# ghnmqdtg/VM-ASR

Hardware: AMD Instinct MI355X
Metric: audio clips/sec (train step) 48kHz n_fft=1024 (higher is better)
Workload: dtype bf16 (autocast over G; scan/STFT f32; MPD f32/bf16x3 MFMA); 1 GPU; vm_asr_48k_MPD.yaml full train step, DIMS 16 d_state 1 n_fft 1024 clip 122640@48k; per_gpu_batch=4, global_batch=4, parallelism=dp1, execution=hipGraph replay, 2 streams, generator_streams=2

## Files before the change

### include/vmasr_hip.h

```cpp
#ifndef VMASR_HIP_H
#define VMASR_HIP_H

#include <stddef.h>
#include <stdint.h>

#ifdef __cplusplus
extern "C" {
#endif

#define VMASR_ABI_VERSION 1

typedef void *vmasr_stream_t;

enum { VMASR_F32 = 0, VMASR_F16 = 1, VMASR_BF16 = 2 };

enum {
    VMASR_OK = 0,
    VMASR_EINVAL = -1,
    VMASR_EALIGN = -2,
    VMASR_ENOSPACE = -3
};

int vmasr_abi_version(void);
const char *vmasr_last_error(void);
// ... 149 lines not shown
                           int32_t k, int32_t stride, int32_t pad, int64_t rows, int32_t dtype, vmasr_stream_t stream);
int vmasr_col2im_kx1_stacked(const void *dcols, void *dx, const int64_t *Ns, const int32_t *Hs, int32_t n, int32_t C, int32_t k, int32_t stride,
                             int32_t pad, int64_t rows, int64_t dx_rows, int32_t dtype, vmasr_stream_t stream);
int vmasr_stack_rows(const void *const *srcs, const int64_t *Ms, int32_t n, void *full, int64_t rows, int64_t row_bytes,
                     vmasr_stream_t stream);


int vmasr_bias_gelu_fwd(float *acc, const float *bias, float *act, int32_t slots, int64_t M, int32_t N, int32_t parts,
                        vmasr_stream_t stream);
int vmasr_weight_prep_split(const float *w, void *out, int32_t n, int32_t N, int32_t K, vmasr_stream_t stream);
int vmasr_weight_transpose(const float *w, void *hi, void *lo, float *out32, int32_t n, int32_t N, int32_t Cin, int32_t k,
                           vmasr_stream_t stream);
int vmasr_sum_parts(const float *parts, float *out, int32_t P, int32_t n, int32_t S, int64_t NK, vmasr_stream_t stream);
int vmasr_gelu_bwd_split(const float *pre, const float *g, void *hi, void *lo, void *cat3, float *db, int32_t slots, int64_t M,
                         int32_t N, vmasr_stream_t stream);
int vmasr_gelu_bwd(const float *pre, const float *g, float *gx, float *db, int32_t slots, int64_t M, int32_t N, vmasr_stream_t stream);

typedef struct vmasr_cg_slot {
    const void *ah, *al;
    const void *bh, *bl;
    float *c0;
    float *c1;
    void *ch, *cl;
    const float *bias;
    int64_t nseq;
    int32_t H;
    int32_t reserved;
} vmasr_cg_slot;
int vmasr_conv_mfma_supported(int32_t Cin, int32_t Cout, int32_t k, int32_t stride);
int vmasr_conv_mfma_supported_launch(int32_t Cin, int32_t Cout, int32_t k, int32_t stride, int32_t n, int64_t rows);
int vmasr_conv_mfma_config(int32_t pass, int32_t Cin, int32_t Cout, int32_t ops, int32_t out[3]);
void vmasr_conv_set_cu_limit(int32_t cus);
int32_t vmasr_conv_get_cu_limit(void);
int vmasr_conv_mfma_fwd(const vmasr_cg_slot *slots, int32_t n, int32_t Cin, int32_t Cout, int32_t k, int32_t stride, int32_t pad,
                        int64_t rows_out, int32_t act, vmasr_stream_t stream);
int vmasr_conv_mfma_dgrad(const vmasr_cg_slot *slots, int32_t n, int32_t Cin, int32_t Cout, int32_t k, int32_t stride, int32_t pad,
                          int64_t rows_in, vmasr_stream_t stream);
int vmasr_conv_f32_fwd(const vmasr_cg_slot *slots, int32_t n, int32_t Cin, int32_t Cout, int32_t k, int32_t stride, int32_t pad,
                       int64_t rows_out, int32_t act, vmasr_stream_t stream);
int vmasr_conv_f32_dgrad(const vmasr_cg_slot *slots, int32_t n, int32_t Cin, int32_t Cout, int32_t k, int32_t stride, int32_t pad,
                         int64_t rows_in, vmasr_stream_t stream);
int vmasr_conv_mfma_wgrad(const vmasr_cg_slot *slots, int32_t n, int32_t Cin, int32_t Cout, int32_t k, int32_t stride, int32_t pad,
                          int32_t splits, vmasr_stream_t stream);
typedef struct vmasr_cg_gelu_bwd {
    const float *pre;
    const signed char *sgn;
    int64_t valid;
    float scale;
    int32_t reserved;
    float *db;
} vmasr_cg_gelu_bwd;
int vmasr_conv_mfma_dgrad_gelu(const vmasr_cg_slot *slots, const vmasr_cg_gelu_bwd *epi, const float *gtok, int32_t n, int32_t Cin, int32_t Cout,
                               int32_t k, int32_t stride, int32_t pad, int64_t rows_in, vmasr_stream_t stream);

int vmasr_wgrad_finish_multi(const float *const *parts, float *const *dws, float *const *dbs, float *const *e1s, float *const *e2s,
                             const int32_t *Ss, const int32_t *Ns, const int32_t *Ks, const int32_t *lds, int32_t n, vmasr_stream_t stream);

int vmasr_linear_f64acc(const float *x, const float *w, const float *bias, float *y, int64_t rows, int32_t out_features,
                        int32_t in_features, vmasr_stream_t stream);

typedef struct vmasr_adamw_item {
    float *p;
    const float *g;
    float *m;
    float *v;
    void *lp;
// ... 246 lines not shown
```

### vm_asr_amd/_lib.py

```python
import ctypes
import os

from . import knobs

_HERE = os.path.dirname(os.path.abspath(__file__))
LIB_PATH = knobs.get("VMASR_LIB") or os.path.join(_HERE, "libvmasr_hip.so")

c_i32, c_i64, c_vp, c_sz = ctypes.c_int32, ctypes.c_int64, ctypes.c_void_p, ctypes.c_size_t

F32, F16, BF16 = 0, 1, 2


class SScanParams(ctypes.Structure):
    _fields_ = (
        [(n, c_i32) for n in ("batch", "dim", "seqlen", "dstate", "n_groups", "n_chunks", "dtype",
                              "delta_softplus")]
        + [(n, c_i64) for n in ("A_d_stride", "A_dstate_stride",
                                "B_batch_stride", "B_group_stride", "B_dstate_stride",
                                "C_batch_stride", "C_group_stride", "C_dstate_stride",
                                "u_batch_stride", "u_d_stride", "delta_batch_stride", "delta_d_stride",
                                "out_batch_stride", "out_d_stride")]
        + [(n, c_vp) for n in ("A_ptr", "B_ptr", "C_ptr", "D_ptr", "u_ptr", "delta_ptr",
                               "delta_bias_ptr", "out_ptr", "x_ptr")]
    )
# ... 86 lines not shown
    "vmasr_bias_gelu_fwd": (ctypes.c_int, [c_vp, c_vp, c_vp, c_i32, c_i64, c_i32, c_i32, c_vp]),
    "vmasr_gelu_bwd": (ctypes.c_int, [c_vp, c_vp, c_vp, c_vp, c_i32, c_i64, c_i32, c_vp]),
    "vmasr_sn_dot_blocks": (c_i32, []),
    "vmasr_sn_stack_fwd": (ctypes.c_int, [c_vp, c_vp, c_i32, c_vp, c_vp, c_vp, c_i32, c_i32, c_i32, c_vp]),
    "vmasr_sn_stack_bwd": (ctypes.c_int, [c_vp, c_vp, c_vp, c_vp, c_vp, c_vp, c_i32, c_vp, c_i32, c_i32, c_i32, c_vp]),
    "vmasr_conv_post_supported": (ctypes.c_int, [c_i32, c_i32]),
    "vmasr_conv_post_fwd": (ctypes.c_int, [c_vp, c_vp, c_vp, c_vp, c_vp, c_vp, c_i32, c_i64, c_i32, c_i32, c_vp]),
    "vmasr_conv_post_bwd": (ctypes.c_int, [c_vp, c_vp, c_vp, c_vp, c_vp, c_vp, c_vp, c_vp, c_i32, c_i64, c_i32, c_i32, c_vp]),
    "vmasr_conv_post_bwd_gelu": (ctypes.c_int, [c_vp] * 16 + [c_i32, c_i64, c_i32, c_i32, c_vp]),
    "vmasr_conv_first_fwd": (ctypes.c_int, [c_vp, c_vp, c_vp, c_i32, c_vp, c_vp, c_vp, c_vp, c_i64, c_vp]),
    "vmasr_conv_first_bwd": (ctypes.c_int, [c_vp, c_vp, c_vp, c_i32, c_vp, c_vp, c_vp, c_vp, c_vp, c_vp, c_i64, c_vp]),
    "vmasr_adamw_chunk": (c_i32, []),
    "vmasr_adamw_step": (ctypes.c_int, [c_vp, c_vp, c_i32, c_i64, c_vp, c_vp, ctypes.c_float, ctypes.c_float, ctypes.c_float, c_vp]),
    "vmasr_masked_l1_blocks": (c_i32, []),
    "vmasr_masked_l1_fwd": (ctypes.c_int, [c_vp, c_vp, c_vp, c_vp, c_vp, c_vp, c_i32, c_i64, c_i64, c_i32, c_vp]),
    "vmasr_masked_l1_bwd": (ctypes.c_int, [c_vp, c_vp, c_vp, c_vp, c_vp, c_i32, c_i64, c_i32, c_vp]),
    "vmasr_lsgan_fwd": (ctypes.c_int, [c_vp, c_vp, c_vp, c_i32, c_vp, c_vp]),
    "vmasr_lsgan_bwd": (ctypes.c_int, [c_vp, c_vp, c_vp, c_vp, c_i32, c_vp, c_vp]),
    "vmasr_masked_l1_bwd_add": (ctypes.c_int, [c_vp, c_vp, c_vp, c_vp, c_vp, c_vp, c_i32, c_i64, c_i32, c_vp]),
    "vmasr_sum_parts": (ctypes.c_int, [c_vp, c_vp, c_i32, c_i32, c_i32, c_i64, c_vp]),
    "vmasr_weight_prep_split": (ctypes.c_int, [c_vp, c_vp, c_i32, c_i32, c_i32, c_vp]),
    "vmasr_weight_transpose": (ctypes.c_int, [c_vp, c_vp, c_vp, c_vp, c_i32, c_i32, c_i32, c_i32, c_vp]),
    "vmasr_gelu_bwd_split": (ctypes.c_int, [c_vp, c_vp, c_vp, c_vp, c_vp, c_vp, c_i32, c_i64, c_i32, c_vp]),
    "vmasr_conv_mfma_supported": (ctypes.c_int, [c_i32, c_i32, c_i32, c_i32]),
    "vmasr_conv_mfma_supported_launch": (ctypes.c_int, [c_i32, c_i32, c_i32, c_i32, c_i32, ctypes.c_int64]),
    "vmasr_conv_mfma_config": (ctypes.c_int, [c_i32, c_i32, c_i32, c_i32, ctypes.POINTER(c_i32)]),
    "vmasr_mark_time": (ctypes.c_int, [c_vp, c_vp]),
    "vmasr_im2col2d_rows": (ctypes.c_int, [c_vp, c_vp] + [c_i32] * 10 + [c_vp, c_i32, c_i32, c_vp]),
    "vmasr_col2im2d_rows": (ctypes.c_int, [c_vp, c_vp] + [c_i32] * 10 + [c_vp, c_i32, c_i32, c_vp]),
    "vmasr_skinny_linear_supported": (ctypes.c_int, [c_i64, c_i32, c_i32]),
    "vmasr_skinny_linear": (ctypes.c_int, [c_vp, c_vp, c_vp, c_vp, c_i64, c_i32, c_i32, c_i64, c_i64, c_i32, c_i32, c_vp]),
    "vmasr_conv_set_cu_limit": (None, [c_i32]),
    "vmasr_conv_get_cu_limit": (c_i32, []),
    "vmasr_conv_mfma_fwd": (ctypes.c_int, [ctypes.POINTER(CgSlot), c_i32, c_i32, c_i32, c_i32, c_i32, c_i32, c_i64, c_i32, c_vp]),
    "vmasr_conv_mfma_dgrad": (ctypes.c_int, [ctypes.POINTER(CgSlot), c_i32, c_i32, c_i32, c_i32, c_i32, c_i32, c_i64, c_vp]),
    "vmasr_conv_f32_fwd": (ctypes.c_int, [ctypes.POINTER(CgSlot), c_i32, c_i32, c_i32, c_i32, c_i32, c_i32, c_i64, c_i32, c_vp]),
    "vmasr_conv_f32_dgrad": (ctypes.c_int, [ctypes.POINTER(CgSlot), c_i32, c_i32, c_i32, c_i32, c_i32, c_i32, c_i64, c_vp]),
    "vmasr_conv_mfma_wgrad": (ctypes.c_int, [ctypes.POINTER(CgSlot), c_i32, c_i32, c_i32, c_i32, c_i32, c_i32, c_i32, c_vp]),
    "vmasr_conv_mfma_dgrad_gelu": (ctypes.c_int, [ctypes.POINTER(CgSlot), ctypes.POINTER(CgGeluBwd), c_vp, c_i32, c_i32, c_i32, c_i32, c_i32,
                                                  c_i32, c_i64, c_vp]),
    "vmasr_wgrad_finish_multi": (ctypes.c_int, [c_vp, c_vp, c_vp, c_vp, c_vp, c_vp, c_vp, c_vp, c_vp, c_i32, c_vp]),
    "vmasr_linear_f64acc": (ctypes.c_int, [c_vp, c_vp, c_vp, c_vp, c_i64, c_i32, c_i32, c_vp]),
    "vmasr_ss2d_glue_supported": (ctypes.c_int, [c_i32, c_i32, c_i32]),
    "vmasr_ss2d_pre_fwd": (ctypes.c_int, [c_vp, c_vp, c_vp, c_i32, c_i32, c_i32, c_i32, c_vp]),
    "vmasr_ss2d_pre_bwd": (ctypes.c_int, [c_vp, c_vp, c_vp, c_vp, c_i32, c_i32, c_i32, c_i32, c_vp]),
    "vmasr_ln_gate_fwd": (ctypes.c_int, [c_vp] * 7 + [c_i32, c_i32, c_i32, ctypes.c_float, c_i32, c_vp]),
    "vmasr_ln_gate_bwd": (ctypes.c_int, [c_vp] * 11 + [c_i32, c_i32, c_i32, c_i32, c_vp]),
    "vmasr_ln_gate_bwd_workspace": (c_i64, [c_i32, c_i32, c_i32, c_i32]),
    "vmasr_ln_gate_bwd_ws": (ctypes.c_int, [c_vp] * 12 + [c_i32, c_i32, c_i32, c_i32, c_vp]),
    "vmasr_ln_gate_pair_supported": (ctypes.c_int, [c_i32, c_i32, c_i32]),
    "vmasr_ln_gate_pair_fwd": (ctypes.c_int, [c_vp] * 8 + [c_i32, c_i32, c_i32, c_i32, ctypes.c_float, c_i32, c_vp]),
    "vmasr_ln_gate_pair_bwd": (ctypes.c_int, [c_vp] * 13 + [c_i32, c_i32, c_i32, c_i32, c_i32, c_vp]),
    "vmasr_ss2d_supported": (ctypes.c_int, [c_i32] * 5),
    "vmasr_ss2d_part_floats": (c_sz, [c_i32] * 4),
    "vmasr_ss2d_fwd": (ctypes.c_int, [ctypes.POINTER(SS2DParams), c_vp]),
    "vmasr_ss2d_bwd": (ctypes.c_int, [ctypes.POINTER(SS2DParams), c_vp]),
    "vmasr_ss2d_deep_supported": (ctypes.c_int, [c_i32] * 5),
    "vmasr_ss2d_deep_waves_per_row": (c_i32, [c_i32, c_i32]),
    "vmasr_ss2d_deep_fwd": (ctypes.c_int, [ctypes.POINTER(SS2DDeepParams), c_vp]),
    "vmasr_ss2d_deep_bwd": (ctypes.c_int, [ctypes.POINTER(SS2DDeepParams), c_vp]),
    "vmasr_set_deterministic": (None, [ctypes.c_int]),
    "vmasr_get_deterministic": (ctypes.c_int, []),
    "vmasr_det_timeouts": (ctypes.c_int64, []),
    "vmasr_prof_enable": (None, [ctypes.c_int]),
    "vmasr_prof_reset": (None, []),
    "vmasr_prof_name": (ctypes.c_char_p, [ctypes.c_int]),
# ... 23 lines not shown
    "vmasr_stem1d_time_tile": (c_i32, []),
    "vmasr_stem1d_channel_group": (c_i32, []),
    "vmasr_stem1d_supported": (ctypes.c_int, [c_i32] * 4),
    "vmasr_stem1d_supported_launch": (ctypes.c_int, [c_i32] * 5 + [c_i64]),
    "vmasr_stem1d_bwd_workspace": (c_sz, [c_i32] * 5 + [c_i64]),
    "vmasr_stem1d_fwd": (ctypes.c_int, [c_vp] * 4 + [c_i32] * 2 + [c_i64] + [c_i32] * 4 + [c_vp]),
    "vmasr_stem1d_bwd": (ctypes.c_int, [c_vp] * 8 + [c_sz] + [c_i32] * 2 + [c_i64] + [c_i32] * 4 + [c_vp]),
    "vmasr_resample_poly": (ctypes.c_int, [c_vp, c_vp, c_vp, c_i32, c_i64, c_i64, c_i32, c_i32, c_i32, c_vp]),
    "vmasr_resample_design_workspace": (c_sz, [c_i32]),
    "vmasr_resample_design": (ctypes.c_int, [c_vp, c_i32, c_i32, c_i32, c_vp, c_sz, c_vp]),
    "vmasr_degrade_batch_workspace": (c_sz, [c_vp, c_i32]),
    "vmasr_degrade_batch": (ctypes.c_int, [c_vp, c_vp, c_vp, c_vp, c_i32, c_i64, c_vp, c_sz, c_vp]),
}

_lib = None


def lib():
    global _lib
    if _lib is None:
        if not os.path.exists(LIB_PATH):
            raise RuntimeError(
                f"{LIB_PATH} is missing: build it with `make -C vm_asr_amd/csrc` "
                "(or __graft_entry__.build()). vm_asr_amd has no CPU fallback.")
        import torch
        l = ctypes.CDLL(LIB_PATH)
        for name, (res, args) in SYMBOLS.items():
            fn = getattr(l, name)
            fn.restype, fn.argtypes = res, args
        if l.vmasr_abi_version() != 1:
            raise RuntimeError("libvmasr_hip.so ABI version mismatch")
        if knobs.get("VMASR_DETERMINISTIC"):
            l.vmasr_set_deterministic(1)
        knobs.warn_undeclared()
        _lib = l
    return _lib


def check(code, what):
    if code != 0:
        msg = lib().vmasr_last_error().decode() or "unknown error"
        raise RuntimeError(f"{what} failed ({code}): {msg}")


def torch_dtype_code(dt):
    import torch
    try:
        return {torch.float32: F32, torch.float16: F16, torch.bfloat16: BF16}[dt]
    except KeyError:
        raise RuntimeError(f"unsupported dtype {dt}: expected float32 / float16 / bfloat16")


def det_mode():
    if knobs.get("VMASR_DETERMINISTIC"):
        return True
    try:
        return bool(lib().vmasr_get_deterministic())
    except (OSError, RuntimeError, AttributeError):
        return False


def current_stream(device):
    import torch
    return ctypes.c_void_p(torch.cuda.current_stream(device).cuda_stream)


# ... 94 lines not shown
```

### vm_asr_amd/csrc/convgemm.hip

```cpp
#include <algorithm>
#include <cstdlib>
#include <type_traits>

#include "common.h"

namespace vmasr {
namespace {

typedef __bf16 bf16x8 __attribute__((ext_vector_type(8)));
typedef float f32x16 __attribute__((ext_vector_type(16)));
typedef float f32x4 __attribute__((ext_vector_type(4)));
typedef unsigned u32x4 __attribute__((ext_vector_type(4)));
typedef __attribute__((address_space(1))) const void *cg_gptr;
typedef __attribute__((address_space(3))) void *cg_lptr;
__device__ uint4 cg_zero_page[4];

constexpr int CG_BM = 128, CG_BN = 128, CG_BK = 32;
constexpr int CG_TILE = CG_BM * CG_BK * 2;
constexpr int CG_STAGE = 4 * CG_TILE;
constexpr int CG_MAXP = 24;

struct CgProb {
    const bf16_t *ah, *al, *bh, *bl;
    float *c0, *c1;
// ... 498 lines not shown
                const bf16x8 ah = cw_frag<RBG, 16>(s, 0, wm * WTM + i * 16, lane);
                const bf16x8 al = cw_frag<RBG, 16>(s + TILE_G, 0, wm * WTM + i * 16, lane);
#pragma unroll
                for (int j = 0; j < TJ; ++j) {
                    acc[i][j] = __builtin_amdgcn_mfma_f32_16x16x32_bf16(al, bh[j], acc[i][j], 0, 0, 0);
                    acc[i][j] = __builtin_amdgcn_mfma_f32_16x16x32_bf16(ah, bl[j], acc[i][j], 0, 0, 0);
                    acc[i][j] = __builtin_amdgcn_mfma_f32_16x16x32_bf16(ah, bh[j], acc[i][j], 0, 0, 0);
                }
            }
        }
        if (!MID_STORE && more) CW_STORE(buf ^ 1);
        __syncthreads();
    }
#undef CW_LOAD
#undef CW_STORE

    const int KC = P.k * Cin;
    float *dw = pr.dw + (size_t)split * Cout * KC;
#pragma unroll
    for (int i = 0; i < TI; ++i)
#pragma unroll
        for (int j = 0; j < TJ; ++j) {
            const int col = kc0 + wn * WTN + j * MF + (MF == 32 ? lr : (lane & 15));
#pragma unroll
            for (int r = 0; r < NR; ++r) {
                const int row = co0 + wm * WTM + i * MF + (MF == 32 ? (r & 3) + 8 * (r >> 2) + 4 * lh : 4 * (lane >> 4) + r);
                dw[(size_t)row * KC + col] = acc[i][j][r];
            }
        }
    __syncthreads();
    }
}

}
}

using namespace vmasr;

namespace {

int g_cg_cu_limit = 0;

int cg_grid(int tiles, size_t smem) {
    if (g_cg_cu_limit <= 0) return tiles;
    const int per_cu = std::max(1, (int)((160 * 1024) / std::max<size_t>(smem, 1)));
    static const int slack = [] { const char *e = getenv("VMASR_CONV_CU_SLACK"); return e ? atoi(e) : 24; }();
    const int cap = std::min(256, g_cg_cu_limit + slack) * per_cu;
    const int rounds = (tiles + cap - 1) / cap;
    const int g = ((tiles + rounds - 1) / rounds + 7) / 8 * 8;
    return std::min(tiles, std::min(g, cap));
}

template <int BM, int BN, int WM, int WN, int MF, int OPS = 0>
int cg_launch_cfg(CgParams &P, int epi, hipStream_t st, int kid, double bytes) {
    int tiles = 0;
    P.ntiles_n = P.NB / BN;
    for (int i = 0; i < P.nprob; ++i) {
        P.prob[i].tile_start = tiles;
        P.prob[i].mtiles = (std::max(P.prob[i].M, P.prob[i].zero_rows) + BM - 1) / BM;
        tiles += P.prob[i].mtiles * P.ntiles_n;
    }
    P.total_tiles = tiles;
    if (tiles == 0) return 0;
    constexpr size_t smem = 2 * (2 * BM * 64 + 2 * BN * 64) + BM * sizeof(int);
    constexpr bool HAS_EPI2 = BN >= 128 && OPS == 0;
    static bool attr_done = false;
// ... 23 lines not shown
    static const int v = [] { const char *e = getenv("VMASR_CONV_TILE"); return e ? atoi(e) : 0; }();
    return v;
}
int env_conv_mfma() {
    static const int v = [] { const char *e = getenv("VMASR_CONV_MFMA"); return e ? atoi(e) : 16; }();
    return v;
}

struct CgConfig {
    int BM, BN, MF;
};
enum { CG_PASS_FWD = 0, CG_PASS_DGRAD = 1, CG_PASS_WGRAD = 2 };

CgConfig cg_config_nt(int NB, int CA, int ops, bool fwd) {
    if (ops) {
        static const int tile = [] { const char *e = getenv("VMASR_CONV_F32_TILE"); return e ? atoi(e) : 128; }();
        if (!fwd) return {256, 32, 32};
        return tile == 256 ? CgConfig{256, 128, 32} : CgConfig{128, 128, 32};
    }
    const int forced = env_conv_tile();
    const int mf = env_conv_mfma() == 16 ? 16 : 32;
    if (NB % 256 == 0 && forced != 128) return {256, 256, mf};
    if (NB % 128 == 0 && CA == 32 && forced != 128) return {256, 128, 16};
    if (NB == 32) return {256, 32, 16};
    return {128, 128, mf};
}

CgConfig cg_config_wgrad(int Cin, int Cout) {
    if (Cout % 256 == 0 && Cin % 256 == 0 && env_conv_tile() != 128) return {256, 256, 16};
    if (Cin == 32) return {128, 32, 16};
    return {128, 128, env_conv_mfma() == 32 ? 32 : 16};
}

CgConfig cg_config(int pass, int Cin, int Cout, int ops) {
    if (pass == CG_PASS_WGRAD) return cg_config_wgrad(Cin, Cout);
    return pass == CG_PASS_FWD ? cg_config_nt(Cout, Cin, ops, true) : cg_config_nt(Cin, Cout, ops, false);
}

int cg_launch(CgParams &P, int epi, hipStream_t st, int kid, double bytes, int ops = 0, bool fwd = true) {
    const CgConfig c = cg_config_nt(P.NB, P.CA, ops, fwd);
    const int key = c.BM * 1000000 + c.BN * 1000 + c.MF;
    if (ops) {
        switch (key) {
            case 256128032: return cg_launch_cfg<256, 128, 4, 2, 32, 1>(P, epi, st, kid, bytes);
            case 256032032: return cg_launch_cfg<256, 32, 8, 1, 32, 1>(P, epi, st, kid, bytes);
            default: return cg_launch_cfg<128, 128, 2, 2, 32, 1>(P, epi, st, kid, bytes);
        }
    }
    switch (key) {
        case 256256016: return cg_launch_cfg<256, 256, 2, 4, 16>(P, epi, st, kid, bytes);
        case 256256032: return cg_launch_cfg<256, 256, 2, 4, 32>(P, epi, st, kid, bytes);
        case 256128016: return cg_launch_cfg<256, 128, 4, 2, 16>(P, epi, st, kid, bytes);
        case 256032016: return cg_launch_cfg<256, 32, 8, 1, 16>(P, epi, st, kid, bytes);
        case 128128032: return cg_launch_cfg<128, 128, 2, 2, 32>(P, epi, st, kid, bytes);
        default: return cg_launch_cfg<128, 128, 2, 2, 16>(P, epi, st, kid, bytes);
    }
}

int64_t cg_fwd_row_bound(int Cin, int Cout, int k, int ops) { return ((int64_t)1 << (ops ? 30 : 31)) / std::max(Cout, k * Cin); }
int64_t cg_dgrad_row_bound(int Cin, int Cout, int k) { return ((int64_t)1 << 31) / std::max(Cin, k * Cout); }
int64_t cg_wgrad_grow_bound(int Cin, int Cout) { return ((int64_t)1 << 31) / std::max(Cout, Cin); }
int64_t cg_wgrad_xrow_bound(int Cin) { return ((int64_t)1 << 31) / Cin; }

}

VMASR_EXPORT void vmasr_conv_set_cu_limit(int32_t cus) { g_cg_cu_limit = cus < 0 ? 0 : cus; }
VMASR_EXPORT int32_t vmasr_conv_get_cu_limit(void) { return g_cg_cu_limit; }

VMASR_EXPORT int vmasr_conv_mfma_supported(int32_t Cin, int32_t Cout, int32_t k, int32_t stride) {
    const bool in_ok = Cin > 0 && (Cin % 128 == 0 || Cin == 32), out_ok = Cout > 0 && Cout % 128 == 0;
    return in_ok && out_ok && k >= 1 && k <= 8 && stride >= 1 && stride <= 3;
}

VMASR_EXPORT int vmasr_conv_mfma_supported_launch(int32_t Cin, int32_t Cout, int32_t k, int32_t stride, int32_t n, int64_t rows) {
    if (!vmasr_conv_mfma_supported(Cin, Cout, k, stride)) return 0;
    if (n < 1 || n > 8 || n * (stride + 1) > CG_MAXP) return 0;
    int64_t bound = std::min(cg_fwd_row_bound(Cin, Cout, k, 0), cg_dgrad_row_bound(Cin, Cout, k));
    bound = std::min(bound, std::min(cg_wgrad_grow_bound(Cin, Cout), cg_wgrad_xrow_bound(Cin)));
    if (Cin == 32) bound = std::min(bound, cg_fwd_row_bound(Cin, Cout, k, 1));
    return rows >= 1 && rows < bound ? 1 : 0;
}

VMASR_EXPORT int vmasr_conv_mfma_config(int32_t pass, int32_t Cin, int32_t Cout, int32_t ops, int32_t out[3]) {
    VMASR_REQUIRE(out && pass >= CG_PASS_FWD && pass <= CG_PASS_WGRAD && (ops == 0 || (ops == 1 && Cin == 32 && pass != CG_PASS_WGRAD)), VMASR_EINVAL,
                  "conv_mfma_config: pass 0..2, ops 0 or 1 (Cin 32, forward / input gradient), out");
    VMASR_REQUIRE(vmasr_conv_mfma_supported(Cin, Cout, 1, 1), VMASR_EINVAL, "conv_mfma_config: unsupported channel counts (Cin %d, Cout %d)", Cin, Cout);
    const CgConfig c = cg_config(pass, Cin, Cout, ops);
    out[0] = c.BM; out[1] = c.BN; out[2] = c.MF;
    return VMASR_OK;
}

namespace {
int cg_fwd(const vmasr_cg_slot *slots, int32_t n, int32_t Cin, int32_t Cout, int32_t k, int32_t stride, int32_t pad, int64_t rows_out,
           int32_t act, vmasr_stream_t stream, int ops) {
    const char *what = ops ? "conv_f32_fwd" : "conv_mfma_fwd";
    VMASR_REQUIRE(slots && n >= 1 && n <= CG_MAXP, VMASR_EINVAL, "%s: 1..%d slots", what, CG_MAXP);
    VMASR_REQUIRE(vmasr_conv_mfma_supported(Cin, Cout, k, stride) && (!ops || Cin == 32), VMASR_EINVAL,
                  "%s: unsupported shape (Cin %d, Cout %d, k %d, stride %d)", what, Cin, Cout, k, stride);
    VMASR_REQUIRE(rows_out % 256 == 0, VMASR_EINVAL, "%s: rows_out must be a multiple of 256", what);
    CgParams P = {};
// ... 88 lines not shown
            p.ah = (const bf16_t *)s.ah; p.al = (const bf16_t *)s.al; p.bh = (const bf16_t *)s.bh; p.bl = (const bf16_t *)s.bl;
            outputs(p);
            p.M = (int)(rows_in - s.nseq * H); p.Q = p.M; p.HA = 1; p.HC = 0;
            p.hq_mul = 0; p.hq_add = 0; p.crow_mul = 1; p.crow_add = (int)(s.nseq * H);
            p.ntaps = 0; p.tap0 = 0; p.tap_step = 1; p.dstep = 0;
            p.zero_rows = 0;
            p.db = nullptr;
        }
        bytes += (double)s.nseq * H1 * Cout * 4 + (double)Cout * k * Cin * 4 + (double)s.nseq * H * Cin * 4;
        if (epi) bytes += (double)s.nseq * H * Cin * ((s.c0 && s.ch ? 4.0 : 0.0) + 4.0 + (epi[i].sgn ? 1.0 : 0.0));
    }
    P.nprob = np;
    return cg_launch(P, epi ? 2 : 0, static_cast<hipStream_t>(stream), VMASR_K_CONV_MFMA_DGRAD, bytes, ops, false);
}

}

VMASR_EXPORT int vmasr_conv_mfma_dgrad(const vmasr_cg_slot *slots, int32_t n, int32_t Cin, int32_t Cout, int32_t k, int32_t stride,
                                       int32_t pad, int64_t rows_in, vmasr_stream_t stream) {
    return cg_dgrad(slots, nullptr, nullptr, n, Cin, Cout, k, stride, pad, rows_in, stream);
}

VMASR_EXPORT int vmasr_conv_f32_dgrad(const vmasr_cg_slot *slots, int32_t n, int32_t Cin, int32_t Cout, int32_t k, int32_t stride,
                                      int32_t pad, int64_t rows_in, vmasr_stream_t stream) {
    return cg_dgrad(slots, nullptr, nullptr, n, Cin, Cout, k, stride, pad, rows_in, stream, 1);
}

VMASR_EXPORT int vmasr_conv_mfma_dgrad_gelu(const vmasr_cg_slot *slots, const vmasr_cg_gelu_bwd *epi, const float *gtok, int32_t n, int32_t Cin,
                                            int32_t Cout, int32_t k, int32_t stride, int32_t pad, int64_t rows_in, vmasr_stream_t stream) {
    VMASR_REQUIRE(epi, VMASR_EINVAL, "conv_mfma_dgrad_gelu: epi is required");
    return cg_dgrad(slots, epi, gtok, n, Cin, Cout, k, stride, pad, rows_in, stream);
}

VMASR_EXPORT int vmasr_conv_mfma_wgrad(const vmasr_cg_slot *slots, int32_t n, int32_t Cin, int32_t Cout, int32_t k, int32_t stride,
                                       int32_t pad, int32_t splits, vmasr_stream_t stream) {
    VMASR_REQUIRE(slots && n >= 1 && n <= 8, VMASR_EINVAL, "conv_mfma_wgrad: 1..8 slots");
    VMASR_REQUIRE(vmasr_conv_mfma_supported(Cin, Cout, k, stride) && splits >= 1 && splits <= 64, VMASR_EINVAL,
                  "conv_mfma_wgrad: unsupported shape (Cin %d, Cout %d, k %d, stride %d, splits %d)", Cin, Cout, k, stride, splits);
    CwParams P = {};
    const CgConfig cfg = cg_config_wgrad(Cin, Cout);
    const bool big = cfg.BM == 256, narrow = cfg.BN == 32;
    const int T = cfg.BM, TK = cfg.BN;
    P.nslots = n; P.splits = splits; P.tiles_co = Cout / T; P.tiles_kc = k * Cin / TK;
    P.Cin = Cin; P.Cout = Cout; P.k = k; P.stride = stride; P.pad = pad;
    double bytes = 0;
    for (int i = 0; i < n; ++i) {
        const vmasr_cg_slot &s = slots[i];
        VMASR_REQUIRE(s.ah && s.al && s.bh && s.bl && s.c0, VMASR_EINVAL, "conv_mfma_wgrad: null tensor in slot %d", i);
        const int64_t H1 = ((int64_t)s.H + 2 * pad - k) / stride + 1, M = s.nseq * H1;
        VMASR_REQUIRE(H1 >= 1 && M < cg_wgrad_grow_bound(Cin, Cout) && s.nseq * (int64_t)s.H < cg_wgrad_xrow_bound(Cin), VMASR_EINVAL,
                      "conv_mfma_wgrad: slot %d too large for 32-bit row offsets", i);
        CwProb &p = P.prob[i];
        p.gh = (const bf16_t *)s.ah; p.gl = (const bf16_t *)s.al; p.xh = (const bf16_t *)s.bh; p.xl = (const bf16_t *)s.bl;
        p.dw = s.c0; p.M = (int)M; p.Q = (int)H1; p.H = s.H;
        const int64_t per = (M + splits - 1) / splits;
        p.mchunk = (int)((per + CW_BR - 1) / CW_BR * CW_BR);
        bytes += (double)M * Cout * 4 + (double)s.nseq * s.H * Cin * 4 + (double)splits * Cout * k * Cin * 4;
    }
    const int tiles = n * splits * P.tiles_co * P.tiles_kc;
    hipStream_t st = static_cast<hipStream_t>(stream);
    if (big) {
        constexpr size_t smem = 2 * 4 * CW_BR * 512;
        static bool attr_done = false;
        if (!attr_done) {
            (void)hipFuncSetAttribute(reinterpret_cast<const void *>(&conv_mfma_wgrad_kernel<256, 256, 2, 4, 16>), hipFuncAttributeMaxDynamicSharedMemorySize, (int)smem);
            attr_done = true;
        }
        VMASR_LAUNCH(VMASR_K_CONV_MFMA_WGRAD, bytes, (conv_mfma_wgrad_kernel<256, 256, 2, 4, 16>), dim3(cg_grid(tiles, smem)), dim3(512), smem, st, P);
    } else if (narrow) {
        VMASR_LAUNCH(VMASR_K_CONV_MFMA_WGRAD, bytes, (conv_mfma_wgrad_kernel<128, 32, 4, 1, 16>), dim3(cg_grid(tiles, 2 * (2 * CW_BR * 256 + 2 * CW_BR * 64))), dim3(256), 2 * (2 * CW_BR * 256 + 2 * CW_BR * 64), st, P);
    } else if (cfg.MF == 32) {
        VMASR_LAUNCH(VMASR_K_CONV_MFMA_WGRAD, bytes, (conv_mfma_wgrad_kernel<128, 128, 2, 2, 32>), dim3(cg_grid(tiles, 2 * 4 * CW_BR * 256)), dim3(256), 2 * 4 * CW_BR * 256, st, P);
    } else {
        VMASR_LAUNCH(VMASR_K_CONV_MFMA_WGRAD, bytes, (conv_mfma_wgrad_kernel<128, 128, 2, 2, 16>), dim3(cg_grid(tiles, 2 * 4 * CW_BR * 256)), dim3(256), 2 * 4 * CW_BR * 256, st, P);
    }
    return check_launch("conv_mfma_wgrad");
}
```

### vm_asr_amd/knobs.py

```python
import os
import warnings
from collections import namedtuple

Knob = namedtuple("Knob", "name kind default values reader doc parse")


def _bad(k, raw, allowed):
    return ValueError(f"{k.name}={raw!r}: expected {allowed}")


def _flag(k, raw):
    if raw == "1":
        return True
    if raw == "0":
        return False
    raise _bad(k, raw, "0 or 1")


def _choice(k, raw):
    if raw in k.values:
        return raw
    raise _bad(k, raw, "one of " + " | ".join(k.values))


# ... 60 lines not shown
    _k("VMASR_LINEAR_F64ACC", "choice", "auto", "fp32 Linear with float64 accumulation: 1 always, 0 never, auto only where no gradient is recorded",
       values=("auto", "0", "1")),
    _k("VMASR_SKINNY", "choice", "1", "streaming kernel for Linear layers of many rows and few features: 1 where it beats the GEMM library, 0 off, "
       "all every supported shape", values=("1", "0", "all")),
    _k("VMASR_SPLITK_CHUNK", "int", 2048, "fewest rows of one K-split of a weight-gradient GEMM; read at import"),
    _k("VMASR_XPROJ_MAX_D", "int", 512, "largest d_inner that takes the x_proj row kernels instead of einsums; read at import"),
    _k("VMASR_FUSED_MLP", "flag", 1, "LayerNorm + Mlp + residual of a VSS block as one operator (mlp.py)"),
    _k("VMASR_FUSED_INPROJ", "flag", 1, "LayerNorm + in_proj + split + SiLU as one operator (inproj.py)"),
    _k("VMASR_FUSED_OUTPROJ", "flag", 1, "out_proj + DropPath + residual as one operator (outproj.py)"),
    _k("VMASR_SS2D_FUSED", "flag", 1, "the d_state-1 SS2D core (x_proj, dt_proj, four-direction scan, merge) as one operator (ss2d_core.py)"),
    _k("VMASR_SS2D_DEEP", "flag", 1, "the deep stages' SS2D core on the row-parallel kernels (ss2d_deep.py)"),
    _k("VMASR_SS2D_GLUE", "flag", 1, "the pre-scan and gated-LayerNorm glue kernels (ss2d_glue.py)"),
    _k("VMASR_SS2D_PAIRS", "flag", 1, "magnitude and phase blocks of equal shape through one gated-LayerNorm launch (ss2d_glue.py)"),
    _k("VMASR_IM2COL2D", "flag", 1, "the generator's 2-D convolutions through the row-major im2col kernel (model.py)"),
    _k("VMASR_STFT_LOSS", "flag", 1, "the multi-resolution STFT loss kernel (loss.py)"),
    _k("VMASR_LSGAN", "flag", 1, "the least-squares GAN loss kernel (loss.py)"),
    _k("VMASR_MPD_BATCHED", "flag", 1, "all period discriminators layer by layer on stacked operands"),
    _k("VMASR_MPD_GEMM", "choice", "bf16x3", "fp32 discriminator GEMMs as bf16x3 MFMA triples, or fp32 library GEMMs", values=("bf16x3", "fp32")),
    _k("VMASR_MPD_CONV", "choice", None, "ONE variable read at two sites.  conv_kx1 (one discriminator at a time; unset = unfold): gemm = the "
       "im2col-free GEMM form for stride 3 and stride 1, s3 = that form for the stride-3 layers only, unfold or mfma = unfold + GEMM.  "
       "Batched path (unset = mfma): mfma = the implicit-GEMM MFMA kernels for the compute-bound layers, gemm / s3 / unfold = not those",
       values=("mfma", "gemm", "s3", "unfold")),
    _k("VMASR_MPD_CONV_L1", "choice", "f32", "the 32 -> 128 layer: f32 exact-fp32 MFMA implicit GEMM, 1 bf16x3 pairs, 0 library GEMMs",
       values=("f32", "1", "0")),
    _k("VMASR_MPD_SPLIT_MIN", "int", 1 << 18, "smallest K * N of a stacked layer that takes the split (hi, lo) GEMM path"),
    _k("VMASR_MPD_KCAT", "flag", 0, "the split GEMM's three products as one GEMM over a concatenated K"),
    _k("VMASR_MPD_FUSE_GELU_BWD", "flag", 1, "the activation backward inside the input-gradient epilogue"),
    _k("VMASR_SN_STACK", "flag", 1, "spectral normalisation, stack and permutation of a layer's weights in one launch"),
    _k("VMASR_STACK_INPUT", "flag", 1, "a layer reads the previous layer's stacked output directly"),
    _k("VMASR_CONV_POST", "flag", 1, "the 1-channel output convolution straight on the stacked maps"),
    _k("VMASR_CONV_FIRST", "flag", 1, "the 1 -> 32 channel input convolution + GELU straight from the folded signals"),
    _k("VMASR_FEAT_TAP", "flag", 1, "a feature map's gradient (next layer's + feature-matching loss's) formed in one pass"),
    _k("VMASR_FEAT_L1", "flag", 1, "the feature-matching loss on the stacked maps in one kernel"),
    _k("VMASR_MSD_CONV", "choice", "hip", "the MSD's strided grouped 1-D convolutions: hip = the exact-fp32 MFMA kernels (csrc/gconv1d.hip), "
       "torch = F.conv1d (A/B measurements, double backward)", values=("hip", "torch"), reader="python:msd"),
    _k("VMASR_MSD_STEM", "choice", "hip", "the MSD's 1 -> hidden stem convolution + GELU: hip = one fused pass that keeps no pre-activation "
       "(csrc/stem1d.hip), torch = F.conv1d + F.gelu (A/B measurements, double backward)", values=("hip", "torch"), reader="python:msd"),
    _k("VMASR_TWO_STREAM", "choice", "1", "the discriminator on a side stream: 1 on, 0 one stream, force also in deterministic mode (test hook)",
       values=("1", "0", "force")),
    _k("VMASR_SHARE_FAKE_PASS", "flag", 1, "one discriminator pass over the fake batch serves both phases of the step"),
    _k("VMASR_GEN_STREAMS", "choice", "auto", "the generator's phase branch on a stream of its own in captured steps: auto where the trainer says so, "
       "1 off, 2 on, 2eager on in eager steps too (debugging aid)", values=("auto", "1", "2", "2eager")),
    _k("VMASR_GEN_LANES", "list", None, "comma list of the segments that leave the main stream (pe,e0..e3,d0..d3,out,ia); unset = all (dev aid)",
       parse=_comma_list),
    _k("VMASR_STEP_VARIANT", "variant", None, "pins the captured step layout: one | lane | lane:<share of the CUs for the discriminator's backward>",
       values=("one", "lane", "lane:0.75"), parse=_step_variant),
    _k("VMASR_SIDE_CUS", "int", None, "CU limit of the discriminator's convolutions beside the generator's backward (and forward unless "
       "VMASR_SIDE_CUS_FWD is set); 0 = no limit; unset = Trainer.side_cu_limits()"),
    _k("VMASR_SIDE_CUS_FWD", "int", None, "the same beside the generator's forward"),
    _k("VMASR_SIDE_CUS_MINC", "int", 0, "the backward limit only for layers at least this wide"),
    _k("VMASR_GRAPH_GC_GUARD", "flag", 1, "no cyclic garbage collection between a graph capture and its first replays"),
    _k("VMASR_PHASE_EVENTS", "flag", 0, "device-clock marks at the step's phase boundaries (tools/phase_probe.py)"),
    _k("VMASR_LN_DEFER", "flag", 1, "LayerNorm's dgamma / dbeta of a whole backward pass reduced in one launch"),
    _k("VMASR_HIP_ADAMW", "flag", 1, "the multi-tensor AdamW kernel on the flat gradient buffers"),
    _k("VMASR_FUSED_ADAMW", "flag", 1, "torch's fused AdamW where the HIP kernel does not apply"),
    _k("VMASR_LP_SHADOWS", "flag", 1, "bf16 shadow copies of the parameters, refreshed by the optimiser kernel"),
    _k("VMASR_LP_SHADOWS_T", "flag", 1, "transposed bf16 shadows of the 2-D weights too"),
    _k("VMASR_RESUME_CONFIG_MISMATCH", "choice", "raise", "a checkpoint written under another configuration: raise or warn", values=("raise", "warn")),
    _k("VMASR_DIST_BACKEND", "str", None, "torch.distributed backend; unset = nccl on a GPU, else gloo"),
    _k("VMASR_DIST_TIMEOUT_S", "int", 600, "process-group timeout in seconds"),
    _k("VMASR_RCCL_TIMEOUT_S", "float", 300.0, "watchdog of a captured collective in seconds (rccl.py)"),
    _k("VMASR_RCCL_DIRECT", "flag", 0, "the trainer's own RCCL communicator outside captures too"),
    _k("VMASR_GRAPH_COLLECTIVES", "flag", 0, "capture the gradient all-reduces into the step's graph"),
    _k("VMASR_OVERLAP_REDUCE", "flag", 1, "asynchronous gradient all-reduces; 0 = strictly between the graphs"),
    _k("VMASR_GRAD_COMM", "choice", "fp32", "wire dtype of the gradient all-reduce: fp32, mpd-bf16 the discriminator's as bf16, bf16 both",
       values=("fp32", "mpd-bf16", "bf16")),
# ... 34 lines not shown
```

Before: 200.6 clips/s.

## Share input tiles across taps in stride-1 conv weight-gradient MFMA kernel

Adds a new weight-gradient kernel for the MPD's stride-1 convolutions. It loads one input tile of CW_BR + 2*(KT-1) rows into LDS and reads every kernel tap from it through transposed LDS reads, so the input is not reloaded for each tap. All k taps accumulate together against one gradient tile using bf16x3 split MFMAs. It is on by default when Cout%256==0, Cin%64==0, k<=5 and stride is 1, with a knob to fall back. The cost is more accumulator registers per thread (TI*KT), which may lower occupancy and adds halo and boundary complexity.

```diff
diff --git a/include/vmasr_hip.h b/include/vmasr_hip.h
--- a/include/vmasr_hip.h
+++ b/include/vmasr_hip.h
@@ -205,6 +205,8 @@
 int vmasr_conv_mfma_config(int32_t pass, int32_t Cin, int32_t Cout, int32_t ops, int32_t out[3]);
 void vmasr_conv_set_cu_limit(int32_t cus);
 int32_t vmasr_conv_get_cu_limit(void);
+void vmasr_conv_set_wgrad_taps(int32_t on);
+int32_t vmasr_conv_get_wgrad_taps(void);
 int vmasr_conv_mfma_fwd(const vmasr_cg_slot *slots, int32_t n, int32_t Cin, int32_t Cout, int32_t k, int32_t stride, int32_t pad,
                         int64_t rows_out, int32_t act, vmasr_stream_t stream);
 int vmasr_conv_mfma_dgrad(const vmasr_cg_slot *slots, int32_t n, int32_t Cin, int32_t Cout, int32_t k, int32_t stride, int32_t pad,
diff --git a/vm_asr_amd/_lib.py b/vm_asr_amd/_lib.py
--- a/vm_asr_amd/_lib.py
+++ b/vm_asr_amd/_lib.py
@@ -142,6 +142,8 @@
     "vmasr_skinny_linear": (ctypes.c_int, [c_vp, c_vp, c_vp, c_vp, c_i64, c_i32, c_i32, c_i64, c_i64, c_i32, c_i32, c_vp]),
     "vmasr_conv_set_cu_limit": (None, [c_i32]),
     "vmasr_conv_get_cu_limit": (c_i32, []),
+    "vmasr_conv_set_wgrad_taps": (None, [c_i32]),
+    "vmasr_conv_get_wgrad_taps": (c_i32, []),
     "vmasr_conv_mfma_fwd": (ctypes.c_int, [ctypes.POINTER(CgSlot), c_i32, c_i32, c_i32, c_i32, c_i32, c_i32, c_i64, c_i32, c_vp]),
     "vmasr_conv_mfma_dgrad": (ctypes.c_int, [ctypes.POINTER(CgSlot), c_i32, c_i32, c_i32, c_i32, c_i32, c_i32, c_i64, c_vp]),
     "vmasr_conv_f32_fwd": (ctypes.c_int, [ctypes.POINTER(CgSlot), c_i32, c_i32, c_i32, c_i32, c_i32, c_i32, c_i64, c_i32, c_vp]),
@@ -231,6 +233,8 @@
             raise RuntimeError("libvmasr_hip.so ABI version mismatch")
         if knobs.get("VMASR_DETERMINISTIC"):
             l.vmasr_set_deterministic(1)
+        if not knobs.get("VMASR_CONV_WGRAD_TAPS"):
+            l.vmasr_conv_set_wgrad_taps(0)
         knobs.warn_undeclared()
         _lib = l
     return _lib
diff --git a/vm_asr_amd/csrc/convgemm.hip b/vm_asr_amd/csrc/convgemm.hip
--- a/vm_asr_amd/csrc/convgemm.hip
+++ b/vm_asr_amd/csrc/convgemm.hip
@@ -554,6 +554,165 @@
     }
 }
 
+template <int ROWB>
+__device__ __forceinline__ int cwt_xoff(const int row, const int ch) {
+    static_assert(ROWB == 128, "x image rows of 64 channels");
+    return row * ROWB + ((ch ^ ((((row >> 1) & 1) | ((row >> 2) & 2)) << 1)) << 4);
+}
+
+template <int ROWB>
+__device__ __forceinline__ bf16x8 cwt_frag(const unsigned char *img, const int ra, const int rb, const int ch, const int sub) {
+    const bf16x4 lo = __builtin_amdgcn_ds_read_tr16_b64_v4bf16((lds_bf16x4 *)(img + cwt_xoff<ROWB>(ra, ch) + sub));
+    const bf16x4 hi = __builtin_amdgcn_ds_read_tr16_b64_v4bf16((lds_bf16x4 *)(img + cwt_xoff<ROWB>(rb, ch) + sub));
+    return __builtin_shufflevector(lo, hi, 0, 1, 2, 3, 4, 5, 6, 7);
+}
+
+template <int BCO, int CC, int WM, int WN, int KT>
+__global__ __launch_bounds__(64 * WM * WN, 2) void conv_mfma_wgrad_taps_kernel(const CwParams P) {
+    constexpr int NT = 64 * WM * WN;
+    constexpr int WTM = BCO / WM, TI = WTM / 16;
+    constexpr int RBG = BCO * 2, RBX = CC * 2;
+    constexpr int XR = CW_BR + 2 * (KT - 1);
+    constexpr int TILE_G = CW_BR * RBG, TILE_X = XR * RBX;
+    constexpr int STAGE = 2 * TILE_G + 2 * TILE_X;
+    constexpr int CG = BCO / 8, CX = CC / 8;
+    constexpr int PG = CW_BR * CG / NT;
+    static_assert(CC == 16 * WN && WTM % 16 == 0 && PG >= 1 && (CW_BR * CG) % NT == 0 && XR * CX <= NT && STAGE % 16 == 0, "tile geometry");
+    extern __shared__ __attribute__((aligned(16))) unsigned char smem[];
+    const int tid = threadIdx.x, lane = tid & 63, wave = tid >> 6;
+    const int wm = wave / WN, wn = wave % WN;
+    const int fr0 = 8 * (lane >> 4) + ((lane & 15) >> 2), fch = 2 * wn + ((lane & 3) >> 1), fsub = 8 * (lane & 1);
+    const bool x_mine = tid < XR * CX;
+    const int x_row = tid / CX, x_ch = tid % CX;
+
+    const int per_slot = P.splits * P.tiles_co * P.tiles_kc;
+#pragma unroll 1
+    for (int tile = blockIdx.x; tile < P.nslots * per_slot; tile += gridDim.x) {
+    const int t_ = xcd_remap(tile, P.nslots * per_slot);
+    const int slot = t_ / per_slot;
+    int rem = t_ - slot * per_slot;
+    const int split = rem / (P.tiles_co * P.tiles_kc);
+    rem -= split * (P.tiles_co * P.tiles_kc);
+    const int tco = rem / P.tiles_kc, tcb = rem - tco * P.tiles_kc;
+    const CwProb &pr = P.prob[slot];
+    const int Cin = P.Cin, Cout = P.Cout;
+    const int co0 = tco * BCO, c0 = tcb * CC;
+    const int mbeg = split * pr.mchunk, mend = min(pr.M, mbeg + pr.mchunk);
+    const int nk = mend > mbeg ? (mend - mbeg + CW_BR - 1) / CW_BR : 0;
+
+    int g_row[PG], g_ch[PG], g_m[PG];
+#pragma unroll
+    for (int i = 0; i < PG; ++i) {
+        const int idx = tid + i * NT;
+        g_row[i] = idx / CG; g_ch[i] = idx % CG;
+        g_m[i] = mbeg + g_row[i];
+    }
+    int ld_m = mbeg, ld_s = mbeg / pr.Q, ld_q = mbeg - ld_s * pr.Q;
+    int ld_b = CW_BR;
+    u32x4 rg_h[PG], rg_l[PG], rx_h, rx_l;
+    bool g_ok[PG], x_ok = false;
+    const u32x4 z4 = {0u, 0u, 0u, 0u};
+
+    f32x4 acc[TI][KT];
+#pragma unroll
+    for (int i = 0; i < TI; ++i)
+#pragma unroll
+        for (int j = 0; j < KT; ++j)
+#pragma unroll
+            for (int r = 0; r < 4; ++r) acc[i][j][r] = 0.f;
+
+#define CWT_LOAD()                                                                                             \
+    do {                                                                                                       \
+        _Pragma("unroll") for (int i = 0; i < PG; ++i) {                                                       \
+            g_ok[i] = g_m[i] < mend;                                                                           \
+            const size_t o_ = (size_t)(g_ok[i] ? g_m[i] : 0) * Cout + co0 + g_ch[i] * 8;                       \
+            rg_h[i] = *reinterpret_cast<const u32x4 *>(pr.gh + o_);                                            \
+            rg_l[i] = *reinterpret_cast<const u32x4 *>(pr.gl + o_);                                            \
+            g_m[i] += CW_BR;                                                                                   \
+        }                                                                                                      \
+        ld_b = min(CW_BR, pr.Q - ld_q);                                                                        \
+        if (x_mine) {                                                                                          \
+            const int left_ = mend - ld_m;                       \
+            const bool second_ = x_row >= ld_b + KT - 1;                  \
+            const int j_ = second_ ? x_row - (ld_b + KT - 1) : x_row;                                          \
+            const int n_ = second_ ? min(CW_BR - ld_b, left_ - ld_b) : min(ld_b, left_);    \
+            const int p_ = (second_ ? 0 : ld_q) + j_ - P.pad;                                                  \
+            x_ok = n_ > 0 && j_ < n_ + P.k - 1 && p_ >= 0 && p_ < pr.H;                                        \
+            const size_t o_ = (size_t)(x_ok ? (ld_s + (second_ ? 1 : 0)) * pr.H + p_ : 0) * Cin + c0 + x_ch * 8; \
+            rx_h = *reinterpret_cast<const u32x4 *>(pr.xh + o_);                                               \
+            rx_l = *reinterpret_cast<const u32x4 *>(pr.xl + o_);                                               \
+        }                                                                                                      \
+        ld_m += CW_BR; ld_q += CW_BR;                                                                          \
+        while (ld_q >= pr.Q) { ld_q -= pr.Q; ++ld_s; }                                                         \
+    } while (0)
+#define CWT_STORE(buf)                                                                                         \
+    do {                                                                                                       \
+        unsigned char *s_ = smem + (buf) * STAGE;                                                              \
+        _Pragma("unroll") for (int i = 0; i < PG; ++i) {                                                       \
+            const int o_ = cw_off<RBG>(g_row[i], g_ch[i]);                                                     \
+            *reinterpret_cast<u32x4 *>(s_ + o_) = g_ok[i] ? rg_h[i] : z4;                                      \
+            *reinterpret_cast<u32x4 *>(s_ + TILE_G + o_) = g_ok[i] ? rg_l[i] : z4;                             \
+        }                                                                                                      \
+        if (x_mine) {                                                                                          \
+            const int o_ = cwt_xoff<RBX>(x_row, x_ch);                                                         \
+            *reinterpret_cast<u32x4 *>(s_ + 2 * TILE_G + o_) = x_ok ? rx_h : z4;                               \
+            *reinterpret_cast<u32x4 *>(s_ + 2 * TILE_G + TILE_X + o_) = x_ok ? rx_l : z4;                      \
+        }                                                                                                      \
+    } while (0)
+
+    if (nk > 0) {
+        CWT_LOAD();
+        CWT_STORE(0);
+    }
+    __syncthreads();
+    for (int kt = 0; kt < nk; ++kt) {
+        const int buf = kt & 1;
+        const bool more = kt + 1 < nk;
+        const int b = ld_b;
+        if (more) CWT_LOAD();
+        const unsigned char *s = smem + buf * STAGE;
+        const int ra = fr0 + (fr0 >= b ? KT - 1 : 0), rb = fr0 + 4 + (fr0 + 4 >= b ? KT - 1 : 0);
+        bf16x8 bh[KT], bl[KT];
+#pragma unroll
+        for (int j = 0; j < KT; ++j) {
+            bh[j] = cwt_frag<RBX>(s + 2 * TILE_G, ra + j, rb + j, fch, fsub);
+            bl[j] = cwt_frag<RBX>(s + 2 * TILE_G + TILE_X, ra + j, rb + j, fch, fsub);
+        }
+#pragma unroll
+        for (int i = 0; i < TI; ++i) {
+            if (i == TI / 2 && more) CWT_STORE(buf ^ 1);
+            const bf16x8 ah = cw_frag<RBG, 16>(s, 0, wm * WTM + i * 16, lane);
+            const bf16x8 al = cw_frag<RBG, 16>(s + TILE_G, 0, wm * WTM + i * 16, lane);
+#pragma unroll
+            for (int j = 0; j < KT; ++j) {
+                acc[i][j] = __builtin_amdgcn_mfma_f32_16x16x32_bf16(al, bh[j], acc[i][j], 0, 0, 0);
+                acc[i][j] = __builtin_amdgcn_mfma_f32_16x16x32_bf16(ah, bl[j], acc[i][j], 0, 0, 0);
+                acc[i][j] = __builtin_amdgcn_mfma_f32_16x16x32_bf16(ah, bh[j], acc[i][j], 0, 0, 0);
+            }
+        }
+        __syncthreads();
+    }
+#undef CWT_LOAD
+#undef CWT_STORE
+
+    const int KC = P.k * Cin;
+    float *dw = pr.dw + (size_t)split * Cout * KC;
+#pragma unroll
+    for (int i = 0; i < TI; ++i)
+#pragma unroll
+        for (int j = 0; j < KT; ++j) {
+            if (j >= P.k) break;
+            const int col = j * Cin + c0 + wn * 16 + (lane & 15);
+#pragma unroll
+            for (int r = 0; r < 4; ++r) {
+                const int row = co0 + wm * WTM + i * 16 + 4 * (lane >> 4) + r;
+                dw[(size_t)row * KC + col] = acc[i][j][r];
+            }
+        }
+    __syncthreads();
+    }
+}
+
 }
 }
 
@@ -643,6 +802,13 @@
     return {128, 128, env_conv_mfma() == 32 ? 32 : 16};
 }
 
+constexpr int CWT_TCO = 128, CWT_CC = 64, CWT_KMAX = 5;
+bool g_cw_taps = true;
+bool cw_taps_enabled() { return g_cw_taps; }
+bool cw_use_taps(int Cin, int Cout, int k, int stride, int64_t min_h1) {
+    return cw_taps_enabled() && stride == 1 && Cout % 256 == 0 && Cin % CWT_CC == 0 && k <= CWT_KMAX && min_h1 >= CW_BR - 1;
+}
+
 CgConfig cg_config(int pass, int Cin, int Cout, int ops) {
     if (pass == CG_PASS_WGRAD) return cg_config_wgrad(Cin, Cout);
     return pass == CG_PASS_FWD ? cg_config_nt(Cout, Cin, ops, true) : cg_config_nt(Cin, Cout, ops, false);
@@ -677,6 +843,9 @@
 
 VMASR_EXPORT void vmasr_conv_set_cu_limit(int32_t cus) { g_cg_cu_limit = cus < 0 ? 0 : cus; }
 VMASR_EXPORT int32_t vmasr_conv_get_cu_limit(void) { return g_cg_cu_limit; }
+
+VMASR_EXPORT void vmasr_conv_set_wgrad_taps(int32_t on) { g_cw_taps = on != 0; }
+VMASR_EXPORT int32_t vmasr_conv_get_wgrad_taps(void) { return cw_taps_enabled() ? 1 : 0; }
 
 VMASR_EXPORT int vmasr_conv_mfma_supported(int32_t Cin, int32_t Cout, int32_t k, int32_t stride) {
     const bool in_ok = Cin > 0 && (Cin % 128 == 0 || Cin == 32), out_ok = Cout > 0 && Cout % 128 == 0;
@@ -831,6 +1000,26 @@
     return cg_dgrad(slots, epi, gtok, n, Cin, Cout, k, stride, pad, rows_in, stream);
 }
 
+namespace {
+template <int KT>
+int cw_launch_taps_kt(CwParams &P, double bytes, hipStream_t st) {
+    constexpr int TCO = CWT_TCO;
+    constexpr size_t smem = 2 * (2 * CW_BR * TCO * 2 + 2 * (CW_BR + 2 * (KT - 1)) * CWT_CC * 2);
+    P.tiles_co = P.Cout / TCO; P.tiles_kc = P.Cin / CWT_CC;
+    const int tiles = P.nslots * P.splits * P.tiles_co * P.tiles_kc;
+    static bool attr_done = false;
+    if (!attr_done) {
+        (void)hipFuncSetAttribute(reinterpret_cast<const void *>(&conv_mfma_wgrad_taps_kernel<TCO, CWT_CC, 2, 4, KT>), hipFuncAttributeMaxDynamicSharedMemorySize, (int)smem);
+        attr_done = true;
+    }
+    VMASR_LAUNCH(VMASR_K_CONV_MFMA_WGRAD, bytes, (conv_mfma_wgrad_taps_kernel<TCO, CWT_CC, 2, 4, KT>), dim3(cg_grid(tiles, std::max<size_t>(smem, 81 * 1024))), dim3(512), smem, st, P);
+    return check_launch("conv_mfma_wgrad");
+}
+int cw_launch_taps(CwParams &P, bool three, double bytes, hipStream_t st) {
+    return three ? cw_launch_taps_kt<3>(P, bytes, st) : cw_launch_taps_kt<5>(P, bytes, st);
+}
+}
+
 VMASR_EXPORT int vmasr_conv_mfma_wgrad(const vmasr_cg_slot *slots, int32_t n, int32_t Cin, int32_t Cout, int32_t k, int32_t stride,
                                        int32_t pad, int32_t splits, vmasr_stream_t stream) {
     VMASR_REQUIRE(slots && n >= 1 && n <= 8, VMASR_EINVAL, "conv_mfma_wgrad: 1..8 slots");
@@ -856,8 +1045,11 @@
         p.mchunk = (int)((per + CW_BR - 1) / CW_BR * CW_BR);
         bytes += (double)M * Cout * 4 + (double)s.nseq * s.H * Cin * 4 + (double)splits * Cout * k * Cin * 4;
     }
+    hipStream_t st = static_cast<hipStream_t>(stream);
+    int64_t min_h1 = INT64_MAX;
+    for (int i = 0; i < n; ++i) min_h1 = std::min<int64_t>(min_h1, P.prob[i].Q);
+    if (cw_use_taps(Cin, Cout, k, stride, min_h1)) return cw_launch_taps(P, k <= 3, bytes, st);
     const int tiles = n * splits * P.tiles_co * P.tiles_kc;
-    hipStream_t st = static_cast<hipStream_t>(stream);
     if (big) {
         constexpr size_t smem = 2 * 4 * CW_BR * 512;
         static bool attr_done = false;
diff --git a/vm_asr_amd/knobs.py b/vm_asr_amd/knobs.py
--- a/vm_asr_amd/knobs.py
+++ b/vm_asr_amd/knobs.py
@@ -116,6 +116,8 @@
     _k("VMASR_CONV_FIRST", "flag", 1, "the 1 -> 32 channel input convolution + GELU straight from the folded signals"),
     _k("VMASR_FEAT_TAP", "flag", 1, "a feature map's gradient (next layer's + feature-matching loss's) formed in one pass"),
     _k("VMASR_FEAT_L1", "flag", 1, "the feature-matching loss on the stacked maps in one kernel"),
+    _k("VMASR_CONV_WGRAD_TAPS", "flag", 1, "the weight gradient of the stride-1 convolutions on the tap-shared tile (csrc/convgemm.hip); 0 = the "
+       "per-tap tile (A/B measurements); read when the library loads, which passes it on (vmasr_conv_set_wgrad_taps)", reader="python:conv"),
     _k("VMASR_MSD_CONV", "choice", "hip", "the MSD's strided grouped 1-D convolutions: hip = the exact-fp32 MFMA kernels (csrc/gconv1d.hip), "
        "torch = F.conv1d (A/B measurements, double backward)", values=("hip", "torch"), reader="python:msd"),
     _k("VMASR_MSD_STEM", "choice", "hip", "the MSD's 1 -> hidden stem convolution + GELU: hip = one fused pass that keeps no pre-activation "
```

Result: no change. 202.0 clips/s (median of 6 runs) (+0.7%).
